# iiscleap/ICL-speech-text-LLM

Hardware: AMD Instinct MI355X
Metric: ICL utterances/sec (whole node), SALMONN+Llama2-7B 5-shot VOXCELEB (higher is better)
Workload: dtype bf16

## Files before the change

icl-speech-text-llm_amd/csrc/gemm256.hip:

```cpp
#include "gemm_common.h"
#include <cstdlib>

using namespace iclg;

#ifndef ICL_EPI_NT
#define ICL_EPI_NT 3
#endif

namespace {

constexpr int T256_REGION = 128 * 128;
constexpr int T256_BUF = 4 * T256_REGION;
constexpr int T256_SMEM = 256 * (256 * 2 + 16);

__device__ __forceinline__ void st16(unsigned short* dst, u32x4 v) {
  if (ICL_EPI_NT & 4) __builtin_nontemporal_store(v, (u32x4*)dst);
  else *(u32x4*)dst = v;
}

__device__ __forceinline__ void rope_rows(const GemmParams& p, const RopeFuse& rf, const char* smem, int pitch, int m0,
                                          int n0, int tid) {
  const int sect = n0 >= rf.v_off ? 2 : (n0 >= rf.k_off ? 1 : 0);
  const int head0 = (n0 - (sect == 2 ? rf.v_off : sect == 1 ? rf.k_off : 0)) >> 7;
  unsigned short* C = (unsigned short*)p.C;
  constexpr int U = 4;
  if (sect == 2) {
    for (int base = tid; base < 256 * 32; base += U * 512) {
      int64_t crow[U];
      if (rf.vc) {
#pragma unroll
        for (int u = 0; u < U; ++u) {
          const int m = min(m0 + ((base + u * 512) >> 5), p.M - 1);
          crow[u] = (int64_t)rf.seq_ids[m] * rf.H * rf.max_len + rf.pos[m];
        }
      }
#pragma unroll
      for (int u = 0; u < U; ++u) {
        const int c = base + u * 512, row = c >> 5, cc = c & 31, m = m0 + row;
        if (m >= p.M) continue;
        const u32x4 v = *(const u32x4*)(smem + row * pitch + cc * 16);
        if (rf.kv_rows_to_c) st16(C + (int64_t)m * p.ldc + n0 + cc * 8, v);
        if (rf.vc) st16(rf.vc + (crow[u] + (int64_t)(head0 + (cc >> 4)) * rf.max_len) * 128 + (cc & 15) * 8, v);
      }
    }
    return;
  }
  const bool to_cache = sect == 1 && rf.kc;
  for (int base = tid; base < 256 * 16; base += U * 512) {
    int ps[U], sq[U];
    u32x4 lo[U], hi[U];
    f32x4 c0[U], c1[U], s0[U], s1[U];
#pragma unroll
    for (int u = 0; u < U; ++u) {
      const int m = min(m0 + ((base + u * 512) >> 4), p.M - 1);
      ps[u] = rf.pos[m];
      sq[u] = to_cache ? rf.seq_ids[m] : 0;
    }
#pragma unroll
    for (int u = 0; u < U; ++u) {
      const int it = base + u * 512, row = it >> 4, hh = (it >> 3) & 1, j = it & 7;
      const char* src = smem + row * pitch + hh * 256 + j * 16;
      lo[u] = *(const u32x4*)src;
      hi[u] = *(const u32x4*)(src + 128);
      const float* cp = rf.cosT + (int64_t)ps[u] * 64 + j * 8;
      const float* sp = rf.sinT + (int64_t)ps[u] * 64 + j * 8;
      c0[u] = *(const f32x4*)cp;
      c1[u] = *(const f32x4*)(cp + 4);
      s0[u] = *(const f32x4*)sp;
      s1[u] = *(const f32x4*)(sp + 4);
    }
#pragma unroll
    for (int u = 0; u < U; ++u) {
      const int it = base + u * 512, row = it >> 4, hh = (it >> 3) & 1, j = it & 7, m = m0 + row;
      if (m >= p.M) continue;
      u32x4 olo, ohi;
      rope_rot8(lo[u], hi[u], c0[u], c1[u], s0[u], s1[u], olo, ohi);
      if (sect == 0 || rf.kv_rows_to_c) {
        unsigned short* dst = C + (int64_t)m * p.ldc + n0 + hh * 128 + j * 8;
        st16(dst, olo);
        st16(dst + 64, ohi);
      }
      if (to_cache) {
        unsigned short* cd = rf.kc + (((int64_t)sq[u] * rf.H + head0 + hh) * rf.max_len + ps[u]) * 128 + j * 8;
        st16(cd, olo);
        st16(cd + 64, ohi);
      }
    }
  }
}

constexpr int T256_OUT_F32 = 16;
template <bool ROPE, int EPI>
__global__ __launch_bounds__(512, 2) void gemm256_bf16_kernel(GemmParams p_in, RopeFuse rf) {
  GemmParams p = p_in;
  p.epi = (p_in.epi & ICL_EPI_BIAS) | (EPI & (ICL_EPI_GELU | ICL_EPI_RESIDUAL | ICL_EPI_SWIGLU));
  p.out_dtype = (EPI & T256_OUT_F32) ? ICL_F32 : ICL_BF16;
  extern __shared__ __attribute__((aligned(16))) char smem[];
  const int tid = threadIdx.x, lane = tid & 63;
  const int wave = __builtin_amdgcn_readfirstlane(tid >> 6);
  const int wr = wave >> 2, wc = wave & 3;
  int tm, tn;
  block_to_tile(p, blockIdx.x, tm, tn);
  const int m0 = tm * 256, n0 = tn * 256;
  int z = blockIdx.z;
  int nk = p.K >> 6, kt0 = 0;
  const bool slab_out = p.split_k > 1;
  if (p.split_k > 1) {
    kt0 = (int)(((int64_t)z * nk) / p.split_k);
    nk = (int)(((int64_t)(z + 1) * nk) / p.split_k) - kt0;
    p.C = p.ws + (int64_t)z * p.M * p.N;
    p.ldc = p.N;
    p.sC = 0;
    p.epi = 0;
    z = 0;
  }
  const __bf16* A = p.A + (int64_t)z * p.sA + (int64_t)kt0 * 64;
  const __bf16* Wk = p.W + (int64_t)kt0 * 64;

  const __bf16* gsrc[2][2][2];
#pragma unroll
  for (int h = 0; h < 2; ++h)
#pragma unroll
    for (int r = 0; r < 2; ++r) {
      const int row = (r * 8 + wave) * 8 + (lane >> 3);
      const int chunk = (lane & 7) ^ ((row >> 1) & 7);
      gsrc[0][h][r] = A + (int64_t)min(m0 + h * 128 + row, p.M - 1) * p.lda + chunk * 8;
      gsrc[1][h][r] = Wk + (int64_t)min(n0 + h * 128 + row, p.N - 1) * p.ldw + chunk * 8;
    }
  auto stage = [&](int bo, int which, int h, int kt) {
    const int64_t koff = (int64_t)min(kt, nk - 1) * 64;
    char* base = smem + bo + (which * 2 + h) * T256_REGION + wave * 1024;
    __builtin_amdgcn_global_load_lds((gptr_t)(gsrc[which][h][0] + koff), (lptr_t)(base), 16, 0, 0);
    __builtin_amdgcn_global_load_lds((gptr_t)(gsrc[which][h][1] + koff), (lptr_t)(base + 8 * 1024), 16, 0, 0);
  };

  const int fr = lane & 15, fq = lane >> 4;
  const int a_base = (wr * 64 + fr) * 128, b_base = (wc * 32 + fr) * 128;
  const int sw0 = ((0 + fq) ^ (fr >> 1)) * 16, sw1 = ((4 + fq) ^ (fr >> 1)) * 16;

  f32x4 acc[2][2][4][2];
#pragma unroll
  for (int a = 0; a < 2; ++a)
#pragma unroll
    for (int b = 0; b < 2; ++b)
#pragma unroll
      for (int i = 0; i < 4; ++i)
#pragma unroll
        for (int j = 0; j < 2; ++j) acc[a][b][i][j] = f32x4{0.f, 0.f, 0.f, 0.f};
  bf16x8 af[4][2], b0f[2][2], b1f[2][2];
  const bool vecp = vec_path_ok(p);
  const bool interior = vecp && (m0 + 256 <= p.M) && (n0 + 256 <= p.N);
  const bool fold_bias = vecp && (p.epi & ICL_EPI_BIAS);
  constexpr bool fold_res = false;

  auto read_a = [&](int bo, int h) {
    const char* r = smem + bo + h * T256_REGION + a_base;
#pragma unroll
    for (int i = 0; i < 4; ++i) {
      af[i][0] = *(const bf16x8*)(r + i * 2048 + sw0);
      af[i][1] = *(const bf16x8*)(r + i * 2048 + sw1);
    }
  };
  auto read_b = [&](int bo, int h, bf16x8 (&bf)[2][2]) {
    const char* r = smem + bo + (2 + h) * T256_REGION + b_base;
#pragma unroll
    for (int j = 0; j < 2; ++j) {
      bf[j][0] = *(const bf16x8*)(r + j * 2048 + sw0);
      bf[j][1] = *(const bf16x8*)(r + j * 2048 + sw1);
    }
  };
  auto mma = [&](f32x4 (&c)[4][2], bf16x8 (&bf)[2][2]) {
    __builtin_amdgcn_s_setprio(1);
#pragma unroll
    for (int kk = 0; kk < 2; ++kk)
#pragma unroll
      for (int i = 0; i < 4; ++i)
#pragma unroll
        for (int j = 0; j < 2; ++j)
          c[i][j] = __builtin_amdgcn_mfma_f32_16x16x32_bf16(bf[j][kk], af[i][kk], c[i][j], 0, 0, 0);
    __builtin_amdgcn_s_setprio(0);
    __builtin_amdgcn_sched_barrier(0);
    __builtin_amdgcn_s_barrier();
    __builtin_amdgcn_sched_barrier(0);
  };
  auto phase_sync = [&](auto n_tag) {
    constexpr int N = decltype(n_tag)::value;
    if constexpr (N == 8) asm volatile("s_waitcnt vmcnt(8)" ::: "memory");
    else if constexpr (N == 6) asm volatile("s_waitcnt vmcnt(6)" ::: "memory");
    else if constexpr (N == 4) asm volatile("s_waitcnt vmcnt(4)" ::: "memory");
    else if constexpr (N == 2) asm volatile("s_waitcnt vmcnt(2)" ::: "memory");
    else asm volatile("s_waitcnt vmcnt(0)" ::: "memory");
    __builtin_amdgcn_sched_barrier(0);
    __builtin_amdgcn_s_barrier();
    __builtin_amdgcn_sched_barrier(0);
  };
  auto tile = [&](int bo, int t, auto mode) {
    constexpr int MODE = decltype(mode)::value;
    const int bx = bo ^ T256_BUF;
    read_a(bo, 0);
    read_b(bo, 0, b0f);
    if constexpr (MODE != 2) stage(bx, 1, 1, t + 1);
    phase_sync(std::integral_constant<int, MODE == 2 ? 2 : 8>{});
    mma(acc[0][0], b0f);
    read_b(bo, 1, b1f);
    if constexpr (MODE != 2) stage(bx, 0, 1, t + 1);
    phase_sync(std::integral_constant<int, MODE == 2 ? 0 : 8>{});
    mma(acc[0][1], b1f);
    read_a(bo, 1);
    if constexpr (MODE == 0) stage(bo, 0, 0, t + 2);
    phase_sync(std::integral_constant<int, MODE == 0 ? 8 : (MODE == 1 ? 6 : 0)>{});
    mma(acc[1][1], b1f);
    if constexpr (MODE == 0) stage(bo, 1, 0, t + 2);
    phase_sync(std::integral_constant<int, MODE == 0 ? 8 : (MODE == 1 ? 4 : 0)>{});
    mma(acc[1][0], b0f);
  };
  using M0_ = std::integral_constant<int, 0>;
  using M1_ = std::integral_constant<int, 1>;
  using M2_ = std::integral_constant<int, 2>;

  f32x4 bias_f[2][2];
  if (fold_res) {
#pragma unroll
    for (int qa = 0; qa < 2; ++qa)
#pragma unroll
      for (int qb = 0; qb < 2; ++qb)
#pragma unroll
        for (int i = 0; i < 4; ++i)
#pragma unroll
          for (int j = 0; j < 2; ++j) {
            const int m = m0 + qa * 128 + wr * 64 + i * 16 + fr, n = n0 + qb * 128 + wc * 32 + j * 16 + fq * 4;
            if (interior || (m < p.M && n < p.N))
              acc[qa][qb][i][j] = *(const f32x4*)((const float*)p.R + (int64_t)z * p.sR + (int64_t)m * p.ldr + n);
          }
  }
  if (fold_bias) {
#pragma unroll
    for (int qb = 0; qb < 2; ++qb)
#pragma unroll
      for (int j = 0; j < 2; ++j) {
        const int n = n0 + qb * 128 + wc * 32 + j * 16 + fq * 4;
        bias_f[qb][j] = (interior || n < p.N) ? *(const f32x4*)(p.bias + n) : f32x4{0.f, 0.f, 0.f, 0.f};
      }
  }
  __builtin_amdgcn_sched_barrier(0);
  stage(0, 0, 0, 0);
  stage(0, 1, 0, 0);
  stage(0, 1, 1, 0);
  stage(0, 0, 1, 0);
  stage(T256_BUF, 0, 0, 1);
  stage(T256_BUF, 1, 0, 1);
  __builtin_amdgcn_sched_barrier(0);
  if (fold_bias) {
#pragma unroll
    for (int qa = 0; qa < 2; ++qa)
#pragma unroll
      for (int qb = 0; qb < 2; ++qb)
#pragma unroll
        for (int i = 0; i < 4; ++i)
#pragma unroll
          for (int j = 0; j < 2; ++j) acc[qa][qb][i][j] = acc[qa][qb][i][j] + bias_f[qb][j];
  }
  phase_sync(std::integral_constant<int, 8>{});
  if (wr == 1) __builtin_amdgcn_s_barrier();
  const int n_steady = nk - 2;
  int t = 0;
  for (; t + 1 < n_steady; t += 2) {
    tile(0, t, M0_{});
    tile(T256_BUF, t + 1, M0_{});
  }
  if (t < n_steady) {
    tile(0, t, M0_{});
    ++t;
  }
  const int bo = (t & 1) ? T256_BUF : 0;
  tile(bo, t, M1_{});
  tile(bo ^ T256_BUF, t + 1, M2_{});
  if (wr == 0) __builtin_amdgcn_s_barrier();

  const int es_out = p.out_dtype == ICL_BF16 ? 2 : 4;
  const bool rows16 = (((uintptr_t)p.C | (uintptr_t)(p.ldc * es_out) | (uintptr_t)(p.sC * es_out)) & 15) == 0;
  const bool has_res = p.epi & ICL_EPI_RESIDUAL;
  const bool res_rows = has_res && p.res_dtype == ICL_F32 && p.out_dtype == ICL_F32 && !(p.epi & ICL_EPI_SWIGLU) &&
                        (((uintptr_t)p.R | (uintptr_t)(p.ldr * 4) | (uintptr_t)(p.sR * 4)) & 15) == 0;
  if (ROPE || (interior && rows16 && (!has_res || res_rows))) {
    const bool swiglu = p.epi & ICL_EPI_SWIGLU;
    const bool obf = p.out_dtype == ICL_BF16;
    const int out_cols = swiglu ? 128 : 256;
    const int es = obf ? 2 : 4;
    const int pitch = out_cols * es + 16;
    const int chunks_per_row = out_cols * es / 16;
    const int64_t c_col0 = swiglu ? (n0 >> 1) : n0;
    const bool one_round = ROPE || obf;
    f32x4 rrA[16], rrB[16];
    auto load_res_rows = [&](int qa_, f32x4 (&rr)[16]) {
      const char* rbase = (const char*)p.R + ((int64_t)z * p.sR + (int64_t)(m0 + qa_ * 128) * p.ldr + n0) * 4;
#pragma unroll
      for (int it = 0; it < 16; ++it) {
        const int c = tid + it * 512, row = c >> 6, cc = c & 63;
        rr[it] = ICL_EPI_NT & 1 ? __builtin_nontemporal_load((const f32x4*)(rbase + (int64_t)row * p.ldr * 4 + cc * 16))
                                : *(const f32x4*)(rbase + (int64_t)row * p.ldr * 4 + cc * 16);
      }
    };
    if (has_res) load_res_rows(0, rrA);
#pragma unroll
    for (int qa = 0; qa < 2; ++qa) {
      if (qa == 0 || !one_round) __syncthreads();
      const int row_off = one_round ? qa * 128 : 0;
#pragma unroll
      for (int qb = 0; qb < 2; ++qb)
#pragma unroll
        for (int i = 0; i < 4; ++i) {
          const int row = row_off + wr * 64 + i * 16 + fr;
          if (swiglu) {
            f32x4 v;
#pragma unroll
            for (int r = 0; r < 4; ++r) v[r] = silu_f(acc[qa][qb][i][0][r]) * acc[qa][qb][i][1][r];
            const int col = qb * 64 + wc * 16 + fq * 4;
            char* dst = smem + row * pitch + col * es;
            if (obf) *(u32x2*)dst = u32x2{pack_bf16x2(v[0], v[1]), pack_bf16x2(v[2], v[3])};
            else *(f32x4*)dst = v;
          } else {
#pragma unroll
            for (int j = 0; j < 2; ++j) {
              f32x4 v = acc[qa][qb][i][j];
              if (p.epi & ICL_EPI_GELU) {
            v = gelu_erf4(v);
              }
              const int col = qb * 128 + wc * 32 + j * 16 + fq * 4;
              char* dst = smem + row * pitch + col * es;
              if (obf) *(u32x2*)dst = u32x2{pack_bf16x2(v[0], v[1]), pack_bf16x2(v[2], v[3])};
              else *(f32x4*)dst = v;
            }
          }
        }
      if (one_round && qa == 0) continue;
      __syncthreads();
      if constexpr (ROPE) {
        rope_rows(p, rf, smem, pitch, m0, n0, tid);
        continue;
      }
      char* cbase = (char*)p.C + ((int64_t)z * p.sC + (int64_t)(m0 + (one_round ? 0 : qa * 128)) * p.ldc + c_col0) * es;
      const int n_chunks = (one_round ? 256 : 128) * chunks_per_row;
      if (has_res) {
        if (qa == 0) load_res_rows(1, rrB);
        f32x4 (&rr)[16] = qa == 0 ? rrA : rrB;
#pragma unroll
        for (int it = 0; it < 16; ++it) {
          const int c = tid + it * 512, row = c >> 6, cc = c & 63;
          const f32x4 v = *(const f32x4*)(smem + row * pitch + cc * 16) + rr[it];
          if (ICL_EPI_NT & 1) __builtin_nontemporal_store(v, (f32x4*)(cbase + (int64_t)row * p.ldc * 4 + cc * 16));
          else *(f32x4*)(cbase + (int64_t)row * p.ldc * 4 + cc * 16) = v;
        }
      } else {
        const int n_iter = n_chunks >> 9;
        u32x4 v[16];
#pragma unroll
        for (int it = 0; it < 16; ++it)
          if (it < n_iter) {
            const int c = tid + it * 512, row = c / chunks_per_row, cc = c - row * chunks_per_row;
            v[it] = *(const u32x4*)(smem + row * pitch + cc * 16);
          }
#pragma unroll
        for (int it = 0; it < 16; ++it)
          if (it < n_iter) {
            const int c = tid + it * 512, row = c / chunks_per_row, cc = c - row * chunks_per_row;
            if ((ICL_EPI_NT & 2) && !slab_out) __builtin_nontemporal_store(v[it], (u32x4*)(cbase + (int64_t)row * p.ldc * es + cc * 16));
            else *(u32x4*)(cbase + (int64_t)row * p.ldc * es + cc * 16) = v[it];
          }
      }
    }
    return;
  } else if (interior) {
    const bool late_res = (p.epi & ICL_EPI_RESIDUAL) && !fold_res;
#pragma unroll
    for (int qa = 0; qa < 2; ++qa) {
      const int mb = m0 + qa * 128 + wr * 64 + fr;
      if (p.epi & ICL_EPI_SWIGLU) {
#pragma unroll
        for (int i = 0; i < 4; ++i)
#pragma unroll
          for (int qb = 0; qb < 2; ++qb) {
            f32x4 v;
#pragma unroll
            for (int r = 0; r < 4; ++r) v[r] = silu_f(acc[qa][qb][i][0][r]) * acc[qa][qb][i][1][r];
            store_out4(p, (int64_t)z * p.sC + (int64_t)(mb + i * 16) * p.ldc + ((n0 + qb * 128 + wc * 32) >> 1) + fq * 4, v);
          }
        continue;
      }
      f32x4 rv[2][4][2];
      if (late_res) {
#pragma unroll
        for (int qb = 0; qb < 2; ++qb)
#pragma unroll
          for (int i = 0; i < 4; ++i)
#pragma unroll
            for (int j = 0; j < 2; ++j)
              rv[qb][i][j] = load_res4(p, (int64_t)z * p.sR + (int64_t)(mb + i * 16) * p.ldr + n0 + qb * 128 + wc * 32 + j * 16 + fq * 4);
      }
#pragma unroll
      for (int qb = 0; qb < 2; ++qb)
#pragma unroll
        for (int i = 0; i < 4; ++i)
#pragma unroll
          for (int j = 0; j < 2; ++j) {
            f32x4 v = acc[qa][qb][i][j];
            if (p.epi & ICL_EPI_GELU) {
            v = gelu_erf4(v);
            }
            if (late_res) v = v + rv[qb][i][j];
            store_out4(p, (int64_t)z * p.sC + (int64_t)(mb + i * 16) * p.ldc + n0 + qb * 128 + wc * 32 + j * 16 + fq * 4, v);
          }
    }
    return;
  }

  GemmParams q = p;
  if (fold_bias) q.epi &= ~ICL_EPI_BIAS;
  if (fold_res) q.epi &= ~ICL_EPI_RESIDUAL;
#pragma unroll
  for (int qa = 0; qa < 2; ++qa)
#pragma unroll
    for (int i = 0; i < 4; ++i) {
      const int m = m0 + qa * 128 + wr * 64 + i * 16 + fr;
#pragma unroll
      for (int qb = 0; qb < 2; ++qb) {
        const int nt = n0 + qb * 128 + wc * 32;
        if (p.epi & ICL_EPI_SWIGLU) {
          epi_store_swiglu(q, z, m, nt, fq * 4, acc[qa][qb][i][0], acc[qa][qb][i][1]);
        } else {
          epi_store4(q, z, m, nt + fq * 4, acc[qa][qb][i][0]);
          epi_store4(q, z, m, nt + 16 + fq * 4, acc[qa][qb][i][1]);
        }
      }
    }
}

template <bool ROPE, int EPI>
int launch256(const GemmParams& p, const dim3& grid, hipStream_t stream, const RopeFuse& rf) {
  auto kern = gemm256_bf16_kernel<ROPE, EPI>;
  if (const int rc = allow_dynamic_lds<gemm256_bf16_kernel<ROPE, EPI>>(T256_SMEM)) return rc;
  hipLaunchKernelGGL(kern, grid, dim3(512), T256_SMEM, stream, p, rf);
  ICL_CHECK_LAUNCH("icl_gemm_bf16(256)");
  return ICL_OK;
}

}

int iclg::launch_tile256(GemmParams& p, int batch, hipStream_t stream, const RopeFuse* rope) {
  p.tiles_m = (p.M + 255) / 256;
  p.tiles_n = (p.N + 255) / 256;
  {
    static const int env_gm = [] { const char* e = getenv("ICL_GEMM_GROUP_M"); return e ? atoi(e) : 0; }();
    static const int env_xs = [] { const char* e = getenv("ICL_GEMM_XCD_SYNC"); return e ? atoi(e) : 1; }();
    const int64_t panel = (int64_t)256 * p.K * 2;
    p.group_m = env_gm > 0 ? env_gm : (int)std::min<int64_t>(6, std::max<int64_t>(1, 8400000 / panel));
    p.xcd_sync = env_xs;
  }
  const dim3 grid(p.tiles_m * p.tiles_n, 1, p.split_k > 1 ? p.split_k : batch);
  if (rope) return launch256<true, 0>(p, grid, stream, *rope);
  const RopeFuse none{};
  constexpr int G = ICL_EPI_GELU, R = ICL_EPI_RESIDUAL, S = ICL_EPI_SWIGLU, F = T256_OUT_F32;
  if (p.split_k > 1) return launch256<false, F>(p, grid, stream, none);
  switch ((p.epi & (G | R | S)) | (p.out_dtype == ICL_F32 ? F : 0)) {
    case 0:         return launch256<false, 0>(p, grid, stream, none);
    case G:         return launch256<false, G>(p, grid, stream, none);
    case R:         return launch256<false, R>(p, grid, stream, none);
    case G | R:     return launch256<false, G | R>(p, grid, stream, none);
    case S:         return launch256<false, S>(p, grid, stream, none);
    case F:         return launch256<false, F>(p, grid, stream, none);
    case F | G:     return launch256<false, F | G>(p, grid, stream, none);
    case F | R:     return launch256<false, F | R>(p, grid, stream, none);
    case F | G | R: return launch256<false, F | G | R>(p, grid, stream, none);
    case F | S:     return launch256<false, F | S>(p, grid, stream, none);
  }
  icl_set_error("icl_gemm_bf16(256): unsupported epilogue combination 0x%x", p.epi);
  return ICL_EINVAL;
}
```

Measured before the change: 142.3.

## Add register-shuffle f32 epilogue using DPP/permlane instead of LDS staging

For f32-output GEMM tiles without rope or swiglu, the accumulator fragments are rearranged across lanes with DPP and permlane swaps so each lane holds contiguous 16-byte row pieces. Residual add and stores then go straight from registers to global memory. This skips the shared-memory round trip and its barriers in the epilogue. The cost is extra cross-lane instructions and more register pressure from double-buffered residual loads.

```diff
diff --git a/icl-speech-text-llm_amd/csrc/gemm256.hip b/icl-speech-text-llm_amd/csrc/gemm256.hip
--- a/icl-speech-text-llm_amd/csrc/gemm256.hip
+++ b/icl-speech-text-llm_amd/csrc/gemm256.hip
@@ -5,6 +5,10 @@
 
 #ifndef ICL_EPI_NT
 #define ICL_EPI_NT 3
+#endif
+
+#ifndef ICL_EPI_F32_REG
+#define ICL_EPI_F32_REG 2
 #endif
 
 namespace {
@@ -84,6 +88,105 @@
         unsigned short* cd = rf.kc + (((int64_t)sq[u] * rf.H + head0 + hh) * rf.max_len + ps[u]) * 128 + j * 8;
         st16(cd, olo);
         st16(cd + 64, ohi);
+      }
+    }
+  }
+}
+
+constexpr int DPP_QUAD_XOR1 = 0xB1, DPP_QUAD_XOR2 = 0x4E;
+constexpr int DPP_ROW_SHL4 = 0x104, DPP_ROW_SHR4 = 0x114, DPP_ROW_ROR8 = 0x128;
+
+template <int CTRL, int BANKS>
+__device__ __forceinline__ float dpp_into(float keep, float src) {
+  return __builtin_bit_cast(float, __builtin_amdgcn_update_dpp(__builtin_bit_cast(int, keep), __builtin_bit_cast(int, src), CTRL,
+                                                               0xf, BANKS, false));
+}
+__device__ __forceinline__ void swap_j_l3(float& a, float& b) {
+  const float na = dpp_into<DPP_ROW_ROR8, 0xC>(a, b), nb = dpp_into<DPP_ROW_ROR8, 0x3>(b, a);
+  a = na, b = nb;
+}
+__device__ __forceinline__ void swap_j_l2(float& a, float& b) {
+  const float na = dpp_into<DPP_ROW_SHR4, 0xA>(a, b), nb = dpp_into<DPP_ROW_SHL4, 0x5>(b, a);
+  a = na, b = nb;
+}
+template <int CTRL>
+__device__ __forceinline__ void swap_j_quad(float& a, float& b, bool hi) {
+  const float out = hi ? a : b;
+  const float in = __builtin_bit_cast(float, __builtin_amdgcn_mov_dpp(__builtin_bit_cast(int, out), CTRL, 0xf, 0xf, false));
+  a = hi ? in : a, b = hi ? b : in;
+}
+template <bool L5>
+__device__ __forceinline__ void swap_j_row(float& a, float& b) {
+  const unsigned ua = __builtin_bit_cast(unsigned, a), ub = __builtin_bit_cast(unsigned, b);
+  unsigned r0, r1;
+  if constexpr (L5) {
+    const auto r = __builtin_amdgcn_permlane32_swap(ua, ub, false, false);
+    r0 = r[0], r1 = r[1];
+  } else {
+    const auto r = __builtin_amdgcn_permlane16_swap(ua, ub, false, false);
+    r0 = r[0], r1 = r[1];
+  }
+  a = __builtin_bit_cast(float, r0), b = __builtin_bit_cast(float, r1);
+}
+
+struct RegEpiLane { int row0, rstep, piece; };
+__device__ __forceinline__ RegEpiLane reg_epi_lane(int lane) {
+  if (ICL_EPI_F32_REG == 1) return {lane & 7, 8, ((lane >> 3) & 1) * 4 + (lane >> 4)};
+  return {((lane >> 3) & 1) * 8 + ((lane >> 4) & 1) * 4 + (lane >> 5), 2, lane & 7};
+}
+__device__ __forceinline__ void reg_epi_exchange(f32x4& x, f32x4& y, int lane) {
+#pragma unroll
+  for (int r = 0; r < 4; ++r) {
+    float a = x[r], b = y[r];
+    if (ICL_EPI_F32_REG == 1) {
+      swap_j_l3(a, b);
+    } else {
+      swap_j_l2(a, b);
+      swap_j_row<false>(a, b);
+      swap_j_quad<DPP_QUAD_XOR1>(a, b, lane & 1);
+      swap_j_row<true>(a, b);
+      swap_j_quad<DPP_QUAD_XOR2>(a, b, lane & 2);
+    }
+    x[r] = a, y[r] = b;
+  }
+}
+
+__device__ __forceinline__ void f32_reg_epilogue(const GemmParams& p, const f32x4 (&acc)[2][2][4][2], int z, int m0, int n0, int wr,
+                                                 int wc, int lane, bool has_res, bool slab_out) {
+  const RegEpiLane at = reg_epi_lane(lane);
+  const int64_t row = m0 + wr * 64 + at.row0, col = n0 + wc * 32 + at.piece * 4;
+  float* cl = (float*)p.C + (int64_t)z * p.sC + row * p.ldc + col;
+  const float* rl = (const float*)p.R + (int64_t)z * p.sR + row * p.ldr + col;
+  const bool nt_store = has_res ? (ICL_EPI_NT & 1) : ((ICL_EPI_NT & 2) && !slab_out);
+  constexpr int QA[4] = {0, 0, 1, 1}, QB[4] = {0, 1, 1, 0};
+  f32x4 rr[2][4][2];
+  auto load_res = [&](int q, f32x4 (&r)[4][2]) {
+#pragma unroll
+    for (int i = 0; i < 4; ++i)
+#pragma unroll
+      for (int s = 0; s < 2; ++s) {
+        const f32x4* src = (const f32x4*)(rl + (int64_t)(QA[q] * 128 + i * 16 + s * at.rstep) * p.ldr + QB[q] * 128);
+        r[i][s] = ICL_EPI_NT & 1 ? __builtin_nontemporal_load(src) : *src;
+      }
+  };
+  if (has_res) load_res(0, rr[0]);
+#pragma unroll
+  for (int q = 0; q < 4; ++q) {
+    if (has_res && q < 3) load_res(q + 1, rr[(q + 1) & 1]);
+#pragma unroll
+    for (int i = 0; i < 4; ++i) {
+      f32x4 v[2] = {acc[QA[q]][QB[q]][i][0], acc[QA[q]][QB[q]][i][1]};
+      if (p.epi & ICL_EPI_GELU) {
+        v[0] = gelu_erf4(v[0]);
+        v[1] = gelu_erf4(v[1]);
+      }
+      reg_epi_exchange(v[0], v[1], lane);
+#pragma unroll
+      for (int s = 0; s < 2; ++s) {
+        if (has_res) v[s] = v[s] + rr[q & 1][i][s];
+        f32x4* dst = (f32x4*)(cl + (int64_t)(QA[q] * 128 + i * 16 + s * at.rstep) * p.ldc + QB[q] * 128);
+        if (nt_store) __builtin_nontemporal_store(v[s], dst);
+        else *dst = v[s];
       }
     }
   }
@@ -282,7 +385,12 @@
   const bool has_res = p.epi & ICL_EPI_RESIDUAL;
   const bool res_rows = has_res && p.res_dtype == ICL_F32 && p.out_dtype == ICL_F32 && !(p.epi & ICL_EPI_SWIGLU) &&
                         (((uintptr_t)p.R | (uintptr_t)(p.ldr * 4) | (uintptr_t)(p.sR * 4)) & 15) == 0;
-  if (ROPE || (interior && rows16 && (!has_res || res_rows))) {
+  const bool row_stores = ROPE || (interior && rows16 && (!has_res || res_rows));
+  constexpr bool reg_epi = ICL_EPI_F32_REG != 0 && !ROPE && (EPI & T256_OUT_F32) && !(EPI & ICL_EPI_SWIGLU);
+  if (reg_epi && row_stores) {
+    f32_reg_epilogue(p, acc, z, m0, n0, wr, wc, lane, has_res, slab_out);
+    return;
+  } else if (row_stores) {
     const bool swiglu = p.epi & ICL_EPI_SWIGLU;
     const bool obf = p.out_dtype == ICL_BF16;
     const int out_cols = swiglu ? 128 : 256;
```

Result: no change. 142.5, median of 6 (+0.1%).
